# tranqkhue/bugcar_image_segmentation

Hardware: AMD Instinct MI355X
Metric: frames/sec ENet 640x480 segmentation -> BEV occupancy grid (synthetic), whole job (higher is better)
Workload: dtype fp32; 1 GPU; config3/5: ENet 640x480 batch 64 per GPU, preprocess + forward + argmax/LUT + fused BEV warp/occgrid (1000x1000 BEV -> 200x200 cells); global_batch=64, per_gpu_batch=64, height=480, width=640, parallelism=frame-sharded dp1, streams_per_gpu=1, hip_graph=True, ranks=1, devices=1, backend=none (one process)

## Files before the change

### bugcar_image_segmentation_amd/_native.py

```python
from __future__ import annotations

import ctypes
import os
import threading
from pathlib import Path

import torch

_PKG = Path(__file__).resolve().parent
LIB_PATH = Path(os.environ.get("BUGSEG_LIB", _PKG / "libbugseg.so"))

OK, EINVAL, ENOMEM, EHIP, EFORMAT, ESTATE = 0, -1, -2, -3, -4, -5
FP32, BF16, F16 = 0, 1, 2
OUT_LOGITS_F32, OUT_CLASS15_U8, OUT_CLASS3_U8, OUT_BINARY_U8 = 0, 1, 2, 3
PRE_ENGINE, PRE_NCHW_F64, PRE_NCHW_F32, PRE_BGR_U8 = 0, 1, 2, 3

EXPORTED = ("bugseg_version", "bugseg_create", "bugseg_destroy", "bugseg_load_weights", "bugseg_num_classes",
            "bugseg_input_bytes", "bugseg_preprocess", "bugseg_nchw_to_input", "bugseg_enet_forward",
            "bugseg_enet_forward_bgr", "bugseg_enet_forward_bgr_ops", "bugseg_enet_forward_bgr_rows",
            "bugseg_bev_source_rows", "bugseg_debug_row_windows", "bugseg_debug_poison_arena",
            "bugseg_debug_stage3_windows", "bugseg_debug_plan_windows", "bugseg_debug_read_block_output",
            "bugseg_debug_pair_walk", "bugseg_debug_pair_plan",
            "bugseg_bev_occgrid", "bugseg_bev_workspace_bytes", "bugseg_bev_occgrid_ws", "bugseg_plan_info", "bugseg_plan_op", "bugseg_plan_launch_op",
            "bugseg_last_error",
            "bugseg_road_filter_workspace_bytes", "bugseg_road_filter", "bugseg_debug_road_filter_ops",
            "bugseg_clahe_workspace_bytes", "bugseg_clahe_bgr", "bugseg_debug_clahe_stage", "bugseg_debug_clahe_table",
            "bugseg_canny_workspace_bytes", "bugseg_canny", "bugseg_debug_canny_stage", "bugseg_confusion",
            "bugseg_bev_warp_image", "bugseg_hough_trig", "bugseg_hough_workspace_bytes", "bugseg_hough_lines",
            "bugseg_debug_hough_stage",
            "bugseg_quad_workspace_bytes", "bugseg_find_quad", "bugseg_quad_moments", "bugseg_debug_quad_stage",
            "bugseg_map_fuse",
            "bugseg_dl_create", "bugseg_dl_destroy", "bugseg_dl_load_weights", "bugseg_dl_set_plan",
            "bugseg_dl_forward", "bugseg_dl_launch_op", "bugseg_dl_read_buffer", "bugseg_dl_last_error",
            "bugseg_dl_set_class_lut", "bugseg_dl_forward_classes", "bugseg_dl_classes_from_logits",
            "bugseg_debug_parse_pack", "bugseg_debug_polar_tables", "bugseg_debug_ctx_info", "bugseg_debug_tile_walk", "bugseg_debug_set_spans", "bugseg_debug_pool_indices",
            "bugseg_dl_debug_check_plan", "bugseg_debug_knobs", "bugseg_dl_debug_knobs", "bugseg_debug_fused_forms")
DL_OP_FIELDS = 32


class BevParams(ctypes.Structure):
    _fields_ = [("M", ctypes.c_double * 9), ("in_rows", ctypes.c_int), ("in_cols", ctypes.c_int),
                ("warp_w", ctypes.c_int), ("warp_h", ctypes.c_int), ("occ_w_px", ctypes.c_int),
                ("occ_h_px", ctypes.c_int), ("occ_w", ctypes.c_int), ("occ_h", ctypes.c_int),
                ("left_x", ctypes.c_int), ("top_y", ctypes.c_int), ("ros_layout", ctypes.c_int),
                ("variant", ctypes.c_int), ("laserscan", ctypes.c_int)]
# ... 58 lines not shown
        lib = ctypes.CDLL(str(p))
        vp, i, sz, cp = ctypes.c_void_p, ctypes.c_int, ctypes.c_size_t, ctypes.c_char_p
        proto = {
            "bugseg_version": (i, []),
            "bugseg_create": (i, [i, i, ctypes.POINTER(vp)]),
            "bugseg_destroy": (i, [vp]),
            "bugseg_load_weights": (i, [vp, vp, sz]),
            "bugseg_num_classes": (i, [vp]),
            "bugseg_input_bytes": (sz, [vp, i, i, i]),
            "bugseg_preprocess": (i, [vp, vp, i, i, i, i, i, i, vp, vp]),
            "bugseg_nchw_to_input": (i, [vp, vp, i, i, i, i, vp, vp]),
            "bugseg_enet_forward": (i, [vp, vp, i, i, i, i, vp, vp]),
            "bugseg_enet_forward_bgr": (i, [vp, vp, i, i, i, i, vp, vp]),
            "bugseg_enet_forward_bgr_ops": (i, [vp, vp, i, i, i, i, vp, i, i, vp]),
            "bugseg_enet_forward_bgr_rows": (i, [vp, vp, i, i, i, i, vp, i, i, i, i, vp]),
            "bugseg_bev_source_rows": (i, [vp, ctypes.POINTER(BevParams), i, i, ctypes.POINTER(i), ctypes.POINTER(i)]),
            "bugseg_debug_row_windows": (i, [i, i, i, i, i, i, vp]),
            "bugseg_debug_poison_arena": (i, [vp, i, vp]),
            "bugseg_debug_stage3_windows": (i, [i, i, i, i, vp, vp]),
            "bugseg_debug_plan_windows": (i, [vp, i, i, vp]),
            "bugseg_debug_read_block_output": (i, [vp, i, vp, sz, vp]),
            "bugseg_debug_pair_walk": (i, [i, vp, i, i, vp]),
            "bugseg_debug_pair_plan": (i, [vp, vp, i]),
            "bugseg_bev_occgrid": (i, [vp, vp, i, ctypes.POINTER(BevParams), vp, vp]),
            "bugseg_bev_workspace_bytes": (sz, [ctypes.POINTER(BevParams), i]),
            "bugseg_bev_occgrid_ws": (i, [vp, vp, i, ctypes.POINTER(BevParams), vp, vp, sz, vp]),
            "bugseg_plan_info": (i, [vp, i, i, i, i, i, ctypes.POINTER(i), ctypes.POINTER(ctypes.c_double),
                                     ctypes.POINTER(ctypes.c_double), ctypes.POINTER(ctypes.c_double)]),
            "bugseg_plan_op": (i, [vp, i, i, i, i, cp, i, ctypes.POINTER(ctypes.c_double),
                                   ctypes.POINTER(ctypes.c_double), ctypes.POINTER(ctypes.c_double)]),
            "bugseg_plan_launch_op": (i, [vp, i, i, i, i, vp]),
            "bugseg_last_error": (cp, [vp]),
            "bugseg_road_filter_workspace_bytes": (sz, [ctypes.POINTER(RoadFilterParams), i]),
            "bugseg_road_filter": (i, [vp, vp, i, ctypes.POINTER(RoadFilterParams), vp, vp, sz, vp]),
            "bugseg_debug_road_filter_ops": (i, [vp, vp, i, ctypes.POINTER(RoadFilterParams), vp, vp, sz, i, i, vp]),
            "bugseg_clahe_workspace_bytes": (sz, [ctypes.POINTER(ClaheParams), i]),
            "bugseg_clahe_bgr": (i, [vp, vp, i, ctypes.POINTER(ClaheParams), vp, vp, sz, vp]),
            "bugseg_debug_clahe_stage": (i, [vp, vp, i, ctypes.POINTER(ClaheParams), i, vp, vp, sz, vp]),
            "bugseg_debug_clahe_table": (i, [i, vp, sz]),
            "bugseg_canny_workspace_bytes": (sz, [ctypes.POINTER(CannyParams), i]),
            "bugseg_canny": (i, [vp, vp, i, ctypes.POINTER(CannyParams), vp, vp, sz, vp]),
            "bugseg_debug_canny_stage": (i, [vp, vp, i, ctypes.POINTER(CannyParams), i, vp, vp, sz, vp]),
            "bugseg_confusion": (i, [vp, vp, vp, i, ctypes.POINTER(ConfusionParams), vp, vp]),
            "bugseg_bev_warp_image": (i, [vp, vp, i, i, ctypes.POINTER(BevParams), i, vp, vp]),
            "bugseg_hough_trig": (i, [ctypes.POINTER(HoughParams), vp]),
            "bugseg_hough_workspace_bytes": (sz, [ctypes.POINTER(HoughParams), i]),
# ... 68 lines not shown
    if lib.bugseg_debug_fused_forms(rows, n) != n:
        raise RuntimeError("bugseg_debug_fused_forms: the form count changed between two calls")
    return [dict(zip(FORM_COLS, rows[k * len(FORM_COLS):(k + 1) * len(FORM_COLS)])) for k in range(n)]


def tile_walk(ntiles: int, grid: int, rev: int) -> list[list[int]]:
    lib = load_library()
    per_max = (ntiles + 7) // 8
    seq = (ctypes.c_int32 * (grid * per_max))()
    count = (ctypes.c_int32 * grid)()
    per = lib.bugseg_debug_tile_walk(ntiles, grid, rev, seq, len(seq), count)
    if per < 0:
        check(per)
    return [list(seq[b * per:b * per + count[b]]) for b in range(grid)]


def row_windows(H: int, W: int, row0: int, row1: int, tile_rows_c64: int = 8, tile_rows_c16: int = 16) -> list[tuple[int, int]]:
    lib = load_library()
    win = (ctypes.c_int32 * 12)()
    check(lib.bugseg_debug_row_windows(H, W, row0, row1, tile_rows_c64, tile_rows_c16, win))
    return [(win[2 * k], win[2 * k + 1]) for k in range(6)]


def stage3_windows(h: int, y0: int, y1: int, blocks) -> list[tuple[int, int]]:
    lib = load_library()
    flat = [int(v) for b in blocks for v in b]
    blk = (ctypes.c_int32 * max(1, len(flat)))(*flat)
    win = (ctypes.c_int32 * max(1, 2 * len(blocks)))()
    m = lib.bugseg_debug_stage3_windows(h, y0, y1, len(blocks), blk, win)
    if m < 0:
        check(m)
    return [(win[2 * k], win[2 * k + 1]) for k in range(m)]


def pair_walk(cands, first_op: int = 0, last_op: int = -1):
    lib = load_library()
    n = len(cands)
    flat = [int(v) for c in cands for v in c]
    cand = (ctypes.c_int32 * max(1, len(flat)))(*flat)
    out = (ctypes.c_int32 * max(1, 2 * n))()
    m = lib.bugseg_debug_pair_walk(n, cand, first_op, n if last_op < 0 else last_op, out)
    if m < 0:
        check(m)
    return m, [(out[2 * k], out[2 * k + 1]) for k in range(n)]


# ... 68 lines not shown

    def bev_source_rows(self, params: BevParams, rows: int, cols: int) -> tuple[int, int]:
        r0, r1 = ctypes.c_int(0), ctypes.c_int(0)
        check(self.lib.bugseg_bev_source_rows(self.h, ctypes.byref(params), rows, cols, ctypes.byref(r0),
                                              ctypes.byref(r1)), self.h)
        return r0.value, r1.value

    def poison_arena(self, byte: int, stream=None) -> None:
        check(self.lib.bugseg_debug_poison_arena(self.h, int(byte), ctypes.c_void_p(stream_handle(stream))), self.h)

    def plan_windows(self, rows) -> list[tuple[int, int, int, int, int]]:
        win = (ctypes.c_int32 * 10)()
        m = self.lib.bugseg_debug_plan_windows(self.h, int(rows[0]), int(rows[1]), win)
        if m < 0:
            check(m, self.h)
        return [tuple(win[5 * k:5 * k + 5]) for k in range(m)]

    def pair_plan(self) -> list[tuple[int, ...]]:
        rows = (ctypes.c_int32 * (8 * 16))()
        m = self.lib.bugseg_debug_pair_plan(self.h, rows, 16)
        if m < 0:
            check(m, self.h)
        return [tuple(rows[8 * k:8 * k + 8]) for k in range(min(m, 16))]

    def read_block_output(self, op: int, out, stream=None) -> None:
        check(self.lib.bugseg_debug_read_block_output(self.h, op, out.data_ptr(), out.numel() * out.element_size(),
                                                      ctypes.c_void_p(stream_handle(stream))), self.h)

    def _stream_ws(self, x, stream, workspace=None, size_fn=None, params=None, B=0):
        st = stream if stream is not None else torch.cuda.current_stream(x.device)
        ws = workspace
        nws = int(size_fn(ctypes.byref(params), B)) if ws is None and size_fn is not None else 0
        if nws:
            with torch.cuda.stream(st):
                ws = torch.empty(nws, dtype=torch.uint8, device=x.device)
        return stream_handle(st), ((0, 0) if ws is None else (ws.data_ptr(), ws.numel() * ws.element_size())), ws

    def _raise_any(self, rc: int) -> None:
        if rc != OK:
            raise BugsegError(rc, self.lib.bugseg_last_error(self.h).decode(errors="replace"))

    def bev(self, seg, B, params: BevParams, out, stream=None):
        sh, w, _keep = self._stream_ws(seg, stream, None, self.lib.bugseg_bev_workspace_bytes, params, B)
        check(self.lib.bugseg_bev_occgrid_ws(self.h, seg.data_ptr(), B, ctypes.byref(params), out.data_ptr(), *w, sh),
              self.h)

# ... 209 lines not shown
```

### bugcar_image_segmentation_amd/csrc/bugseg_runtime.cpp

```cpp
#include <climits>
#include <cmath>
#include <cstdio>
#include <cstring>
#include <string>
#include <vector>
#include <algorithm>
#include <cstdlib>
#include <mutex>
#include <variant>

#include "bugseg_internal.h"
#include "../../include/bugseg.h"

using namespace bugseg;

namespace {
std::mutex g_occ_mu;
struct OccKey { int dev; const void *f; int threads; size_t lds; int val; };
std::vector<OccKey> g_occ;
int current_device() {
    int d = 0;
    return hipGetDevice(&d) == hipSuccess ? d : 0;
}
}
// ... 21 lines not shown
    const int dev = current_device();
    std::lock_guard<std::mutex> lk(g_occ_mu);
    for (const OccKey &k : g_occ)
        if (k.dev == dev && k.f == f && k.threads == -1) return hipSuccess;
    hipError_t e = hipFuncSetAttribute(f, hipFuncAttributeMaxDynamicSharedMemorySize, 160 * 1024);
    if (e == hipSuccess) g_occ.push_back({dev, f, -1, 0, 1});
    return e;
}

bool bugseg::read_knobs(Knobs &k, std::string &err) {
    k = Knobs();
    auto read = [&](const char *var, int &field, long lo, long hi) {
        const char *v = std::getenv(var);
        if (!v || !*v) return true;
        char *end = nullptr;
        const long n = std::strtol(v, &end, 10);
        const bool ok = (*v == '-' || (*v >= '0' && *v <= '9')) && !*end && n >= lo && n <= hi && !(&field == &k.bev_f && n == 3);
        if (ok) field = (int)n;
        else err = std::string(var) + "=" + v + ": not a decimal integer this knob takes (" + std::to_string(lo) + " to " + std::to_string(hi) + ")";
        return ok;
    };
#define X(name, field, def, lo, hi) if (!read("BUGSEG_" #name, k.field, lo, hi)) return false;
    BUGSEG_KNOBS(X)
#undef X
    return true;
}
int bugseg::dump_knobs(const Knobs *k, char *buf, int len, std::string &err) {
    Knobs now;
    if (!k && !read_knobs(now, err)) return BUGSEG_EINVAL;
    if (!k) k = &now;
    std::string s;
#define X(name, field, def, lo, hi) s += "BUGSEG_" #name "=" + std::to_string(k->field) + "\n";
    BUGSEG_KNOBS(X)
#undef X
    if (!buf || len <= (int)s.size()) {
        err = "the knob dump needs a buffer of " + std::to_string(s.size() + 1) + " bytes";
        return BUGSEG_EINVAL;
    }
    std::memcpy(buf, s.c_str(), s.size() + 1);
    return BUGSEG_OK;
}

int bugseg::range_weight_exp(double m) {
    if (!(m > 0) || !std::isfinite(m)) return 0;
    int e = 0;
    (void)std::frexp(m, &e);
// ... 61 lines not shown
    int fwd_odd = 0;
    double layer() const { return layer_bytes >= 0 ? layer_bytes : bytes; }
    const ConvLaunch *conv() const { return std::get_if<ConvLaunch>(&l); }
    const BneckLaunch *bneck() const { return std::get_if<BneckLaunch>(&l); }
    const UpLaunch *up() const { return std::get_if<UpLaunch>(&l); }
    bool regular(int C, int h) const {
        const BneckLaunch *b = bneck();
        return b && b->C == C && !b->asym && b->cin == 0 && b->a.dt == 1 && b->a.phases == 1 && b->a.H == h;
    }
    bool up_on(int h) const { return up() && up()->a.h == h; }
    bool epi(int e) const { return conv() && conv()->epi == e; }
    bool class_kernel() const { return conv() && conv()->cls; }
};

struct Binding {
    const void *in = nullptr;
    bool bgr = false;
    int out_kind = 0; void *out = nullptr;
};

constexpr int WIN_OPS = 6;
struct WinOp { int y0 = 0, y1 = 0, var = 0, tr = 0, te = 1, tiles_x = 0, tiles_y = 0; Launch l; };
constexpr int S3_OPS = 2;
struct WinPlan {
    int row0 = 0, row1 = 0; WinOp op[WIN_OPS]; int ns3 = 0; WinOp s3[S3_OPS];
    const Launch *launch_of(int i, int n) const {
        const int k = i - (n - WIN_OPS);
        return k >= 0 ? &op[k].l : -k - 1 < ns3 ? &s3[-k - 1].l : nullptr;
    }
};

struct PairCand { bool ok = false; int h = 0, w = 0, in = -1, out = -1; };
std::vector<int> pair_firsts(const std::vector<PairCand> &c) {
    std::vector<int> f;
    for (size_t i = 0; i + 1 < c.size(); ++i) {
        const PairCand &p = c[i], &q = c[i + 1];
        if (p.ok && q.ok && p.h == q.h && p.w == q.w && p.in >= 0 && p.out >= 0 && p.in != p.out && q.in == p.out && q.out == p.in) {
            f.push_back((int)i);
            ++i;
        }
    }
    return f;
}
enum { PA_PLAIN = 0, PA_PAIR = 1, PA_SKIP = 2, PA_LONE_FIRST = 3, PA_LONE_SECOND = 4 };
void pair_actions(int n, const std::vector<int> &firsts, int first_op, int last_op, int *act, int *flip) {
    for (int k = 0; k < n; ++k) { act[k] = PA_PLAIN; flip[k] = 0; }
    for (const int i : firsts) {
        if (i < 0 || i + 1 >= n) continue;
        const bool both = first_op <= i && i + 1 < last_op;
        act[i] = both ? PA_PAIR : PA_LONE_FIRST;
        act[i + 1] = both ? PA_SKIP : PA_LONE_SECOND;
        for (int k = i + 2; k < n; ++k) flip[k] ^= 1;
    }
}
struct PairOp {
    int first = 0, flip = 0;
    BneckPairArgs args{};
    BneckGuardArgs ga{}, gb{};
};

struct Plan {
    int B = 0, H = 0, W = 0;
    std::vector<Op> ops;
    std::vector<int> firsts;
    std::vector<PairOp> pairs;
    std::vector<WinPlan> wins;
    size_t act_bytes = 0;
    float *words = nullptr;
    size_t words_bytes = 0;
    void *arena = nullptr;
    size_t arena_bytes = 0;
    bool pinned = false;
    std::vector<unsigned char *> idx;
    std::vector<size_t> idx_bytes;
    bool cls_ok = false, cls_on = false;
    Launch cls_fused, cls_fused_fwd;
    Binding bound;
};

inline int round_up(int v, int m) { return (v + m - 1) / m * m; }
inline int pow2_nr(int npad) {
    int nr = npad / 16;
    int p = 1;
    while (p < nr) p <<= 1;
    return p;
}

}

// ... 944 lines not shown
    a.cw = l.w; a.cbias = l.bias; a.ncls = l.ncls; a.csw = l.rg.sw[0];
    a.cls_bytes = (uint32_t)((size_t)l.B * l.Hout * l.Wout);
    return f;
}

Launch flipped(const Launch &l, unsigned char *const X[2]) {
    Launch f = l;
    auto mv = [&](auto *&p) {
        using P = std::remove_reference_t<decltype(p)>;
        if ((const void *)p == X[0]) p = (P)X[1];
        else if ((const void *)p == X[1]) p = (P)X[0];
    };
    if (ConvLaunch *c = std::get_if<ConvLaunch>(&f)) { mv(c->a.in); mv(c->a.out); mv(c->a.res); }
    else if (UpLaunch *u = std::get_if<UpLaunch>(&f)) { mv(u->a.x); mv(u->a.out); }
    else if (BneckLaunch *b = std::get_if<BneckLaunch>(&f)) { mv(b->a.x); mv(b->a.out); mv(b->a.xin); }
    return f;
}

void build_pairs(bugseg_ctx *ctx, unsigned char *const X[2], unsigned char *spare, size_t spare_bytes) {
    Plan &pl = ctx->plan;
    const int n = (int)pl.ops.size();
    pl.pairs.clear();
    pl.firsts.clear();
    const Knobs &k = ctx->knobs;
    if (ctx->prec == PREC_F32 && !k.no_fuse && k.bneck_variant < 0 && k.bneck_variant_c64 < 0) {
        auto buf = [&](const void *p) { return p == X[0] ? 0 : p == X[1] ? 1 : -1; };
        std::vector<PairCand> c((size_t)n);
        for (int i = 0; i < n - WIN_OPS; ++i) {
            const BneckLaunch *b = pl.ops[(size_t)i].bneck();
            if (!b || !pl.ops[(size_t)i].regular(64, b->a.H) || b->a.tr || b->cls || b->win || b->var < 0 || b->var > 2) continue;
            if (b->a.x_bytes > spare_bytes) continue;
            c[(size_t)i] = PairCand{true, b->a.H, b->a.W, buf(b->a.x), buf(b->a.out)};
        }
        pl.firsts = pair_firsts(c);
    }
    std::vector<int> act((size_t)n), flip((size_t)n);
    pair_actions(n, pl.firsts, 0, n, act.data(), flip.data());
    for (int i = 0; i < n; ++i) {
        Op &op = pl.ops[(size_t)i];
        op.fwd = flip[(size_t)i] ? flipped(op.l, X) : op.l;
        op.fwd_odd = (op.pos & 1) ^ flip[(size_t)i];
    }
    int th, tw, threads;
    size_t lds;
    bneck_pair_shape(th, tw, threads, lds);
    for (int i = 0; i < n; ++i) {
// ... 81 lines not shown
    pl.act_bytes = total - al(words_bytes);
    pl.wins.clear();
    return true;
}

template <typename F>
void row_windows(int H, int row0, int row1, F tile_rows, int (*win)[2]) {
    const int h2 = H / 2, h4 = H / 4, h8 = H / 8;
    int a = row0, b = row1;
    auto set = [&](int k) { win[k][0] = a; win[k][1] = b; };
    auto halve = [&](int h) { a >>= 1; b = std::min((b + 1) >> 1, h); };
    auto grow = [&](int h) { a = std::max(a - 1, 0); b = std::min(b + 1, h); };
    auto tiles = [&](int k, int h) {
        const int t = std::max(1, tile_rows(k, a, b));
        b = std::min(a + (b - a + t - 1) / t * t, h);
    };
    halve(h2); set(5);
    b = std::min(b + 1, h2);
    tiles(4, h2); set(4); grow(h2);
    halve(h4); set(3);
    tiles(2, h4); set(2); grow(h4);
    tiles(1, h4); set(1); grow(h4);
    halve(h8); set(0);
}

struct S3Desc { int asym = 0, d = 1, rd = 0, rows_full = 0; };
template <typename F>
int stage3_windows(int h, int y0, int y1, int n, const S3Desc *blk, F tile_rows, int (*win)[2]) {
    int a = std::max(y0, 0), b = std::min(y1, h), k = 0;
    for (; k < n; ++k) {
        const S3Desc &q = blk[k];
        if (a >= b || (a == 0 && b == h) || q.d < 1) break;
        int e = b, run;
        if (q.rd) {
            if (q.asym || (q.d & (q.d - 1))) break;
            run = b - a;
        } else {
            if (q.d != 1) break;
            const int t = tile_rows(k, a, b);
            if (t <= 0) break;
            run = (b - a + t - 1) / t * t;
            e = std::min(a + run, h);
        }
        if (run >= q.rows_full) break;
        win[k][0] = a; win[k][1] = e;
        const int reach = q.asym ? 2 : q.d;
// ... 36 lines not shown
        if (w.row0 == row0 && w.row1 == row1) return &w;
    const int n = (int)pl.ops.size(), H = pl.H;
    if (n < WIN_OPS + 1 || pl.cls_ok) return nullptr;
    const Op *o = &pl.ops[(size_t)(n - WIN_OPS)];
    if (!(o[0].up_on(H / 8) && o[1].regular(64, H / 4) && o[2].regular(64, H / 4) && o[3].up_on(H / 4) &&
          o[4].regular(16, H / 2) && o[5].class_kernel() && o[5].conv()->a.Hg == H / 2))
        return nullptr;
    auto s3b = [&](int k) { return n - WIN_OPS - 1 - k >= 0 ? std::get_if<BneckLaunch>(&pl.ops[(size_t)(n - WIN_OPS - 1 - k)].fwd) : nullptr; };
    auto form = [&](const BneckLaunch &q, int rows, bool s3, WinOp &r) {
        auto built = [&](int v) { return !s3 || bneck_slots_per_cu(ctx->knobs, ctx->prec, q.C, q.asym, v, false, 0, true) > 0; };
        int ty = 0, tx = 0, tr = 0, rd = 0;
        int v = pick_bneck_variant(ctx, q.C, q.asym, 1, pl.B, rows, q.a.W, ty, tx, tr, rd);
        if (v < 0 || rd || (s3 && (tr || !built(v)))) { v = q.var; tr = s3 ? 0 : q.a.tr; }
        if (!built(v)) return 0;
        int th, tw, nw;
        bneck_shape(q.C, v, th, tw, nw, nullptr);
        r.var = v; r.tr = tr;
        r.te = tr ? tw : th;
        r.tiles_x = tr ? (q.a.W + th - 1) / th : (q.a.W + tw - 1) / tw;
        return r.te;
    };
    WinPlan w;
    w.row0 = row0; w.row1 = row1;
    int win[WIN_OPS][2];
    row_windows(H, row0, row1, [&](int k, int need0, int need1) { return form(*o[k].bneck(), need1 - need0, false, w.op[k]); }, win);
    for (int k = 0; k < WIN_OPS; ++k) {
        WinOp &r = w.op[k];
        r.y0 = win[k][0]; r.y1 = win[k][1];
        r.tiles_y = (r.y1 - r.y0 + r.te - 1) / r.te;
        r.l = narrow(o[k].fwd, r, false, row0, row1);
    }
    if (ctx->knobs.row_window_s3) {
        S3Desc blk[S3_OPS];
        int nb = 0, th[S3_OPS], tw, nw;
        for (; nb < S3_OPS; ++nb) {
            const BneckLaunch *q = s3b(nb);
            if (!(q && q->C == 128 && q->cin == 0 && q->a.H == H / 8 && q->a.W == o[0].up()->a.w)) break;
            S3Desc &d = blk[nb];
            bneck_shape(128, q->var, th[nb], tw, nw, &d.rd);
            d.asym = q->asym; d.d = q->a.dt;
            d.rows_full = d.rd ? q->a.phases * q->a.tiles_y * th[nb] : q->a.tr ? 0 : q->a.tiles_y * th[nb];
            if (d.rd && bneck_slots_per_cu(ctx->knobs, ctx->prec, 128, false, q->var, false, 0, true) <= 0) d.rows_full = 0;
        }
        int w3[S3_OPS][2];
        w.ns3 = stage3_windows(H / 8, w.op[0].y0, w.op[0].y1, nb, blk,
                               [&](int k, int need0, int need1) { return form(*s3b(k), need1 - need0, true, w.s3[k]); }, w3);
        for (int k = 0; k < w.ns3; ++k) {
            const BneckLaunch &q = *s3b(k);
            WinOp &r = w.s3[k];
            r.y0 = w3[k][0]; r.y1 = w3[k][1];
            if (blk[k].rd) {
                r.var = q.var; r.tr = 0; r.te = th[k]; r.tiles_x = 1;
                r.tiles_y = ((r.y1 - r.y0 + q.a.dt - 1) / q.a.dt + r.te - 1) / r.te;
// ... 259 lines not shown
        }
    }
    hipError_t e = launch_preprocess(a, (hipStream_t)stream);
    if (e != hipSuccess) return fail(ctx, BUGSEG_EHIP, std::string("preprocess launch: ") + hipGetErrorString(e));
    return BUGSEG_OK;
}

int bugseg_nchw_to_input(bugseg_ctx *ctx, const void *x, int is_f64, int B, int H, int W, void *out, void *stream) {
    if (!ctx || !x || !out) return fail(ctx, BUGSEG_EINVAL, "NULL argument");
    if (B <= 0 || H <= 0 || W <= 0) return fail(ctx, BUGSEG_EINVAL, "bad shape");
    DeviceGuard g(ctx->device);
    NchwArgs a{x, is_f64 ? 1 : 0, B, H, W, ctx->prec, out};
    hipError_t e = launch_nchw_to_input(a, (hipStream_t)stream);
    if (e != hipSuccess) return fail(ctx, BUGSEG_EHIP, std::string("layout launch: ") + hipGetErrorString(e));
    return BUGSEG_OK;
}

static hipError_t dispatch(const bugseg_ctx *c, const ConvLaunch &l, hipStream_t s) { return launch_conv(c->prec, l.nr, l.epi, l.a, s, l.cls); }
static hipError_t dispatch(const bugseg_ctx *c, const UpLaunch &l, hipStream_t s) { return launch_up(c->prec, l.cin, l.it, l.cout, l.a, s); }
static hipError_t dispatch(const bugseg_ctx *c, const BneckLaunch &l, hipStream_t s) {
    return l.cls ? launch_bneck_cls(c->knobs, c->prec, l.a, s)
                 : launch_bneck(c->knobs, c->prec, l.C, l.asym, l.var, l.a, s, l.cin, l.win);
}
static int walk_rev(const bugseg_ctx *ctx, int i, bool fwd) {
    const Op &o = ctx->plan.ops[(size_t)i];
    const int order = ctx->knobs.tile_order;
    return order == 2 ? 1 : order == 1 ? (fwd ? o.fwd_odd : o.pos & 1) : 0;
}
static unsigned long long *span_slots(const bugseg_ctx *ctx, int i) {
    return ctx->spans && i < ctx->spans_ops ? ctx->spans + 512 * (size_t)i : nullptr;
}

static hipError_t issue(const bugseg_ctx *ctx, Launch &l, int rev, unsigned long long *span, hipStream_t s) {
    return std::visit([&](auto &r) {
        r.a.span = span;
        r.a.rev = rev;
        return dispatch(ctx, r, s);
    }, l);
}

static void bind(const bugseg_ctx *ctx, const Binding &b, bool first, bool last, Launch &l) {
    ConvLaunch *c = std::get_if<ConvLaunch>(&l);
    if (first && c) {
        c->epi = b.bgr ? EPI_INIT_BGR : EPI_INIT;
        c->a.in = b.in;
        c->a.nlut = b.bgr ? (const double *)((const unsigned char *)ctx->dev_luts + 32) : nullptr;
        c->a.naff_on = b.bgr && ctx->naff_on;
        std::memcpy(c->a.naff, ctx->naff, sizeof(ctx->naff));
        c->a.rg.amax_in = b.bgr ? nullptr : ctx->plan.words;
        c->a.rg.amax_static = b.bgr ? ctx->norm_amax : 0.f;
// ... 1 lines not shown
    if (!last) return;
    const uint8_t *luts = (const uint8_t *)ctx->dev_luts;
    const bool logits = b.out_kind == BUGSEG_OUT_LOGITS_F32;
    uint8_t *cls_out = logits ? nullptr : (uint8_t *)b.out;
    const int lut_kind = b.out_kind == BUGSEG_OUT_CLASS3_U8 ? 1 : b.out_kind == BUGSEG_OUT_BINARY_U8 ? 2 : 0;
    const uint8_t *lut = lut_kind ? luts + 16 * (lut_kind - 1) : nullptr;
    if (BneckLaunch *f = std::get_if<BneckLaunch>(&l)) {
        f->a.cls_out = cls_out; f->a.lut = lut; f->a.lut_kind = lut_kind;
    } else if (c) {
        c->a.cls_out = cls_out; c->a.lut = lut; c->a.lut_kind = lut_kind;
        c->a.logits_out = logits ? (float *)b.out : nullptr;
    }
}

static hipError_t launch_op(const bugseg_ctx *ctx, int i, hipStream_t s, const WinPlan *wp = nullptr, bool fwd = false) {
    const Plan &pl = ctx->plan;
    const int n = (int)pl.ops.size();
    if (pl.cls_on && i + 1 == n) return hipSuccess;
    const bool fused = pl.cls_on && i + 2 == n;
    const Launch *pick = wp ? wp->launch_of(i, n) : nullptr;
    if (!pick) pick = fused ? (fwd ? &pl.cls_fused_fwd : &pl.cls_fused) : fwd ? &pl.ops[(size_t)i].fwd : &pl.ops[(size_t)i].l;
    Launch l = *pick;
    bind(ctx, pl.bound, i == 0, fused || i + 1 == n, l);
    return issue(ctx, l, walk_rev(ctx, i, fwd), span_slots(ctx, i), s);
}

static hipError_t launch_pair(const bugseg_ctx *ctx, const PairOp &p, hipStream_t s) {
    const int i = p.first;
    const BneckLaunch &A = std::get<BneckLaunch>(ctx->plan.ops[(size_t)i].fwd), &Bk = std::get<BneckLaunch>(ctx->plan.ops[(size_t)i + 1].fwd);
    BneckPairArgs a = p.args;
    BneckArgs fa = A.a, fb = Bk.a;
    a.a.rev = fa.rev = walk_rev(ctx, i, true);
    a.a.span = span_slots(ctx, i); fa.span = nullptr;
    fb.rev = walk_rev(ctx, i + 1, true);
    fb.span = span_slots(ctx, i + 1);
    hipError_t e = launch_bneck_pair(ctx->knobs, a, s);
    if (e == hipSuccess) e = launch_bneck_guarded(ctx->knobs, A.var, fa, p.ga, s);
    if (e == hipSuccess) e = launch_bneck_guarded(ctx->knobs, Bk.var, fb, p.gb, s);
    return e;
}

static int enet_forward(bugseg_ctx *ctx, const void *in, bool bgr, int B, int H, int W, int out_kind, void *out,
                        void *stream, int first_op = 0, int last_op = -1, int row0 = 0, int row1 = 0) {
    if (!ctx || !in || !out) return fail(ctx, BUGSEG_EINVAL, "NULL argument");
    if (!ctx->loaded) return fail(ctx, BUGSEG_ESTATE, "no weights loaded");
    if (out_kind < BUGSEG_OUT_LOGITS_F32 || out_kind > BUGSEG_OUT_BINARY_U8) return fail(ctx, BUGSEG_EINVAL, "bad out_kind");
    DeviceGuard g(ctx->device);
    std::string why;
    if (!build_plan(ctx, B, H, W, why, stream)) return fail(ctx, BUGSEG_EINVAL, why);
    Plan &pl = ctx->plan;
    if (stream_capturing(stream)) pl.pinned = true;
    pl.bound = Binding{in, bgr, out_kind, out};
    const int nops = (int)pl.ops.size();
    if (last_op < 0 || last_op > nops) last_op = nops;
    if (first_op < 0 || first_op > last_op) return fail(ctx, BUGSEG_EINVAL, "bad op range");
    if (pl.words && first_op == 0) {
        hipError_t e = hipMemsetAsync(pl.words, 0, pl.words_bytes, (hipStream_t)stream);
        if (e == hipSuccess && !bgr) e = launch_amax((const float *)in, (size_t)B * H * W * 8, pl.words, (hipStream_t)stream);
        if (e != hipSuccess) return fail(ctx, BUGSEG_EHIP, std::string("range words: ") + hipGetErrorString(e));
    }
    pl.cls_on = pl.cls_ok && out_kind != BUGSEG_OUT_LOGITS_F32 && first_op <= nops - 2 && last_op == nops;
    const WinPlan *wp = window_plan(ctx, row0, row1);
    std::vector<int> act(2 * (size_t)nops);
    pair_actions(nops, pl.firsts, first_op, last_op, act.data(), act.data() + nops);
    for (int i = first_op; i < last_op; ++i) {
        hipError_t e = hipSuccess;
        switch (act[(size_t)i]) {
        case PA_SKIP: break;
        case PA_PAIR:
            e = launch_pair(ctx, pl.pairs[(size_t)(std::lower_bound(pl.firsts.begin(), pl.firsts.end(), i) - pl.firsts.begin())], (hipStream_t)stream);
            if (e != hipSuccess) return fail(ctx, BUGSEG_EHIP, "pair launch " + std::to_string(i) + ": " + hipGetErrorString(e));
            break;
        default:
            e = launch_op(ctx, i, (hipStream_t)stream, wp, true);
            if (e != hipSuccess) return fail(ctx, BUGSEG_EHIP, "conv launch " + std::to_string(i) + ": " + hipGetErrorString(e));
        }
    }
    return BUGSEG_OK;
}

int bugseg_enet_forward(bugseg_ctx *ctx, const void *in, int B, int H, int W, int out_kind, void *out, void *stream) {
    return enet_forward(ctx, in, false, B, H, W, out_kind, out, stream);
}

int bugseg_enet_forward_bgr(bugseg_ctx *ctx, const uint8_t *bgr, int B, int H, int W, int out_kind, void *out,
                            void *stream) {
    return enet_forward(ctx, bgr, true, B, H, W, out_kind, out, stream);
}

// ... 417 lines not shown
    }
    return per;
}

int bugseg_debug_fused_forms(int32_t *rows, int n_rows) {
    if (n_rows < 0 || (!rows && n_rows > 0)) return fail(nullptr, BUGSEG_EINVAL, "fused forms: NULL rows");
    const int nb = bneck_form_rows(rows, n_rows);
    const int left = n_rows > nb ? n_rows - nb : 0;
    return nb + up_form_rows(left ? rows + (size_t)nb * FORM_COLS : nullptr, left);
}

int bugseg_debug_row_windows(int H, int W, int row0, int row1, int tile_rows_c64, int tile_rows_c16, int32_t *win) {
    (void)W;
    if (!win) return fail(nullptr, BUGSEG_EINVAL, "NULL argument");
    if (H <= 0 || H % 8 || W <= 0 || W % 8) return fail(nullptr, BUGSEG_EINVAL, "H and W must be positive multiples of 8");
    if (row0 < 0 || row1 > H || row0 >= row1) return fail(nullptr, BUGSEG_EINVAL, "row windows: 0 <= row0 < row1 <= H");
    if (tile_rows_c64 <= 0 || tile_rows_c16 <= 0) return fail(nullptr, BUGSEG_EINVAL, "row windows: tile rows must be positive");
    int w[WIN_OPS][2];
    row_windows(H, row0, row1, [&](int k, int, int) { return k == 4 ? tile_rows_c16 : tile_rows_c64; }, w);
    for (int k = 0; k < WIN_OPS; ++k) { win[2 * k] = w[k][0]; win[2 * k + 1] = w[k][1]; }
    return BUGSEG_OK;
}

int bugseg_debug_poison_arena(bugseg_ctx *ctx, int byte, void *stream) {
    if (!ctx) return fail(ctx, BUGSEG_EINVAL, "NULL ctx");
    Plan &pl = ctx->plan;
    if (!pl.arena) return fail(ctx, BUGSEG_ESTATE, "no forward has run");
    DeviceGuard g(ctx->device);
    hipError_t e = hipMemsetAsync(pl.arena, byte & 255, pl.act_bytes, (hipStream_t)stream);
    if (e != hipSuccess) return fail(ctx, BUGSEG_EHIP, std::string("poison arena: ") + hipGetErrorString(e));
    return BUGSEG_OK;
}

int bugseg_debug_stage3_windows(int h, int y0, int y1, int n, const int32_t *blk, int32_t *win) {
    if (h <= 0 || y0 < 0 || y0 >= y1 || y1 > h || n < 0 || n > 16 || (n && (!blk || !win)))
        return fail(nullptr, BUGSEG_EINVAL, "bad stage-3 walk");
    S3Desc d[16];
    int te[16], w[16][2];
    for (int k = 0; k < n; ++k) {
        d[k].asym = blk[5 * k]; d[k].d = blk[5 * k + 1]; d[k].rd = blk[5 * k + 2]; d[k].rows_full = blk[5 * k + 3];
        te[k] = blk[5 * k + 4];
    }
    const int m = stage3_windows(h, y0, y1, n, d, [&](int k, int, int) { return te[k]; }, w);
    for (int k = 0; k < m; ++k) { win[2 * k] = w[k][0]; win[2 * k + 1] = w[k][1]; }
    return m;
}
// ... 172 lines not shown
```

### bugcar_image_segmentation_amd/csrc/knobs.h

```cpp
#pragma once
#include <string>

#ifndef BUGSEG_TILE_ORDER_DEFAULT
#define BUGSEG_TILE_ORDER_DEFAULT 1
#endif

namespace bugseg {

#define BUGSEG_KNOBS(X) \
    X(F32_RANGE, f32_range, 1, 0, 1) X(NO_PAIR, no_pair, 0, 0, 1) X(NO_FUSE, no_fuse, 0, 0, 1) \
    X(BNECK_VARIANT, bneck_variant, -1, 0, 5) X(BNECK_VARIANT_C128, bneck_variant_c128, -1, 0, bneck_variants(128) - 1) \
    X(BNECK_VARIANT_C64, bneck_variant_c64, -1, 0, bneck_variants(64) - 1) \
    X(BNECK_VARIANT_C16, bneck_variant_c16, -1, 0, bneck_variants(16) - 1) X(BNECK_VARIANT_ASYM, bneck_variant_asym, -1, 0, 5) \
    X(BNECK2, bneck2, 0, 0, 1) X(TILE_ORDER, tile_order, BUGSEG_TILE_ORDER_DEFAULT, 0, 2) X(CLS_FUSE, cls_fuse, 0, 0, 1) \
    X(CLS_CONV, cls_conv, 0, 0, 1) X(ROW_WINDOW_S3, row_window_s3, 1, 0, 1) X(INIT_TABLE, init_table, 0, 0, 1) \
    X(INIT_POOL_SCAN, init_pool_scan, 0, 0, 1) X(BNECK_GRID, bneck_grid, 0, INT_MIN, INT_MAX) \
    X(BEV_F, bev_f, 0, 1, 4)  X(BEV_FG, bev_fg, 0, 0, INT_MAX) X(BEV_BAND, bev_band, 1, 0, 1) \
    X(BEV_FB, bev_fb, 1, 1, 2) X(BEV_NEAR_FIRST, bev_near_first, 0, 0, 1) \
    X(DL_GEMM, dl_gemm, 1, 0, 1) X(DL_G128, dl_g128, 1, 0, 1) X(DL_IG, dl_ig, 1, 0, 1) X(DL_IG64, dl_ig64, 1, 0, 1) \
    X(DL_GTM, dl_gtm, -1, 0, 1) X(DL_GROUP, dl_group, 1, 0, 1)

struct Knobs {
#define X(name, field, def, lo, hi) int field = def;
    BUGSEG_KNOBS(X)
#undef X
};

bool read_knobs(Knobs &k, std::string &err);
int dump_knobs(const Knobs *k, char *buf, int len, std::string &err);

}
```

### include/bugseg.h

```cpp
#ifndef BUGSEG_H
#define BUGSEG_H

#include <stddef.h>
#include <stdint.h>

#ifdef __cplusplus
extern "C" {
#endif

typedef struct bugseg_ctx bugseg_ctx;

enum {
    BUGSEG_OK = 0,
    BUGSEG_EINVAL = -1,
    BUGSEG_ENOMEM = -2,
    BUGSEG_EHIP = -3,
    BUGSEG_EFORMAT = -4,
    BUGSEG_ESTATE = -5
};

enum { BUGSEG_FP32 = 0, BUGSEG_BF16 = 1, BUGSEG_F16 = 2 };

enum {
    BUGSEG_OUT_LOGITS_F32 = 0,
// ... 155 lines not shown

int bugseg_confusion(bugseg_ctx *ctx, const uint8_t *pred_dev, const uint8_t *gt_dev, int B,
                     const bugseg_confusion_params *p, int64_t *acc_dev, void *stream);

int bugseg_plan_info(bugseg_ctx *ctx, int B, int H, int W, int out_kind, int bgr_input, int *n_launches,
                     double *alg_bytes, double *plan_bytes, double *flops);

int bugseg_plan_op(bugseg_ctx *ctx, int B, int H, int W, int op, char *kernel, int kernel_len, double *alg_bytes,
                   double *plan_bytes, double *flops);
int bugseg_plan_launch_op(bugseg_ctx *ctx, int B, int H, int W, int op, void *stream);

const char *bugseg_last_error(const bugseg_ctx *ctx);

int bugseg_debug_parse_pack(const void *blob, size_t bytes, int precision, int *ncls);
int bugseg_debug_polar_tables(int w, int h, int variant, int32_t *fmap, size_t fmap_n, int32_t *imap, size_t imap_n,
                              int *pw, int *ph);
int bugseg_debug_tile_walk(int ntiles, int grid, int rev, int32_t *seq, size_t seq_n, int32_t *count);
int bugseg_debug_row_windows(int H, int W, int row0, int row1, int tile_rows_c64, int tile_rows_c16, int32_t *win);
int bugseg_debug_stage3_windows(int h, int y0, int y1, int n, const int32_t *blk, int32_t *win);
int bugseg_debug_plan_windows(bugseg_ctx *ctx, int row0, int row1, int32_t *win);
int bugseg_debug_read_block_output(bugseg_ctx *ctx, int op, void *dst_dev, size_t bytes, void *stream);
int bugseg_debug_pair_walk(int n, const int32_t *cand, int first_op, int last_op, int32_t *out);
int bugseg_debug_pair_plan(bugseg_ctx *ctx, int32_t *rows, int cap);
int bugseg_debug_poison_arena(bugseg_ctx *ctx, int byte, void *stream);
int bugseg_debug_ctx_info(const bugseg_ctx *ctx, int what, int arg);
int bugseg_debug_knobs(const bugseg_ctx *ctx, char *buf, int len);
int bugseg_debug_fused_forms(int32_t *rows, int n_rows);
int bugseg_debug_set_spans(bugseg_ctx *ctx, void *spans, int n_ops);
int bugseg_debug_pool_indices(bugseg_ctx *ctx, int B, int H, int W, int block, void *dst, size_t bytes, int *idx_cs,
                              void *stream);

#define BUGSEG_DL_OP_FIELDS 32
typedef struct bugseg_dl bugseg_dl;

int bugseg_dl_create(int device, int precision, bugseg_dl **out);
int bugseg_dl_destroy(bugseg_dl *dl);
int bugseg_dl_load_weights(bugseg_dl *dl, const void *blob, size_t bytes);
int bugseg_dl_set_plan(bugseg_dl *dl, const int32_t *ops, int nops, const uint64_t *buf_bytes, int nbufs,
                       int B, int Hc, int Wc);
int bugseg_dl_forward(bugseg_dl *dl, const uint8_t *rgb_dev, int B, int H, int W, int64_t *out_dev, void *stream);
int bugseg_dl_set_class_lut(bugseg_dl *dl, const uint8_t *lut, int n);
int bugseg_dl_forward_classes(bugseg_dl *dl, const uint8_t *img_dev, int bgr, int B, int H, int W, uint8_t *seg_dev,
                              int row0, int row1, void *stream);
int bugseg_dl_classes_from_logits(bugseg_dl *dl, int B, int H, int W, uint8_t *seg_dev, int row0, int row1,
                                  void *stream);
int bugseg_dl_launch_op(bugseg_dl *dl, int op, void *stream);
// ... 11 lines not shown
```

Before: 23770 frames/s.

## Fuse two decoder bottlenecks into a paired launch inside the row-window plan

Extends the row-windowed (BEV source rows) forward plan so that two consecutive decoder bottleneck ops (ops 1 and 2 of the window) run as one fused pair kernel. The intermediate goes through a spare buffer, and the following ops have their ping-pong buffers flipped. The row window for the pair is rounded up to the pair tile height, and the upstream window is widened to cover it. The aim is to cut one launch and the round trip of the intermediate activation through global memory, at the cost of some extra rows computed from the rounding and more complex buffer aliasing.

```diff
diff --git a/bugcar_image_segmentation_amd/_native.py b/bugcar_image_segmentation_amd/_native.py
--- a/bugcar_image_segmentation_amd/_native.py
+++ b/bugcar_image_segmentation_amd/_native.py
@@ -20,7 +20,7 @@
             "bugseg_enet_forward_bgr", "bugseg_enet_forward_bgr_ops", "bugseg_enet_forward_bgr_rows",
             "bugseg_bev_source_rows", "bugseg_debug_row_windows", "bugseg_debug_poison_arena",
             "bugseg_debug_stage3_windows", "bugseg_debug_plan_windows", "bugseg_debug_read_block_output",
-            "bugseg_debug_pair_walk", "bugseg_debug_pair_plan",
+            "bugseg_debug_pair_walk", "bugseg_debug_pair_plan", "bugseg_debug_row_windows_pair", "bugseg_debug_decoder_pair",
             "bugseg_bev_occgrid", "bugseg_bev_workspace_bytes", "bugseg_bev_occgrid_ws", "bugseg_plan_info", "bugseg_plan_op", "bugseg_plan_launch_op",
             "bugseg_last_error",
             "bugseg_road_filter_workspace_bytes", "bugseg_road_filter", "bugseg_debug_road_filter_ops",
@@ -125,6 +125,8 @@
             "bugseg_debug_read_block_output": (i, [vp, i, vp, sz, vp]),
             "bugseg_debug_pair_walk": (i, [i, vp, i, i, vp]),
             "bugseg_debug_pair_plan": (i, [vp, vp, i]),
+            "bugseg_debug_row_windows_pair": (i, [i, i, i, i, i, i, i, vp]),
+            "bugseg_debug_decoder_pair": (i, [vp, i, i, vp]),
             "bugseg_bev_occgrid": (i, [vp, vp, i, ctypes.POINTER(BevParams), vp, vp]),
             "bugseg_bev_workspace_bytes": (sz, [ctypes.POINTER(BevParams), i]),
             "bugseg_bev_occgrid_ws": (i, [vp, vp, i, ctypes.POINTER(BevParams), vp, vp, sz, vp]),
@@ -239,6 +241,14 @@
     return [(win[2 * k], win[2 * k + 1]) for k in range(6)]
 
 
+def row_windows_pair(H: int, W: int, row0: int, row1: int, tile_rows_c64: int = 8, tile_rows_c16: int = 16,
+                     pair_rows: int = 12) -> list[tuple[int, int]]:
+    lib = load_library()
+    win = (ctypes.c_int32 * 14)()
+    check(lib.bugseg_debug_row_windows_pair(H, W, row0, row1, tile_rows_c64, tile_rows_c16, pair_rows, win))
+    return [(win[2 * k], win[2 * k + 1]) for k in range(7)]
+
+
 def stage3_windows(h: int, y0: int, y1: int, blocks) -> list[tuple[int, int]]:
     lib = load_library()
     flat = [int(v) for b in blocks for v in b]
@@ -353,6 +363,13 @@
         if m < 0:
             check(m, self.h)
         return [tuple(rows[8 * k:8 * k + 8]) for k in range(min(m, 16))]
+
+    def decoder_pair(self, rows) -> tuple[int, ...] | None:
+        info = (ctypes.c_int32 * 8)()
+        m = self.lib.bugseg_debug_decoder_pair(self.h, int(rows[0]), int(rows[1]), info)
+        if m < 0:
+            check(m, self.h)
+        return tuple(info) if m else None
 
     def read_block_output(self, op: int, out, stream=None) -> None:
         check(self.lib.bugseg_debug_read_block_output(self.h, op, out.data_ptr(), out.numel() * out.element_size(),
diff --git a/bugcar_image_segmentation_amd/csrc/bugseg_runtime.cpp b/bugcar_image_segmentation_amd/csrc/bugseg_runtime.cpp
--- a/bugcar_image_segmentation_amd/csrc/bugseg_runtime.cpp
+++ b/bugcar_image_segmentation_amd/csrc/bugseg_runtime.cpp
@@ -67,6 +67,7 @@
     };
 #define X(name, field, def, lo, hi) if (!read("BUGSEG_" #name, k.field, lo, hi)) return false;
     BUGSEG_KNOBS(X)
+    BUGSEG_KNOBS_UNLISTED(X)
 #undef X
     return true;
 }
@@ -174,12 +175,20 @@
 constexpr int WIN_OPS = 6;
 struct WinOp { int y0 = 0, y1 = 0, var = 0, tr = 0, te = 1, tiles_x = 0, tiles_y = 0; Launch l; };
 constexpr int S3_OPS = 2;
+struct PairOp {
+    int first = 0, flip = 0;
+    BneckPairArgs args{};
+    BneckGuardArgs ga{}, gb{};
+};
 struct WinPlan {
     int row0 = 0, row1 = 0; WinOp op[WIN_OPS]; int ns3 = 0; WinOp s3[S3_OPS];
     const Launch *launch_of(int i, int n) const {
         const int k = i - (n - WIN_OPS);
         return k >= 0 ? &op[k].l : -k - 1 < ns3 ? &s3[-k - 1].l : nullptr;
     }
+    bool paired = false;
+    PairOp pair;
+    int py0 = 0, py1 = 0, pth = 0, ptw = 0;
 };
 
 struct PairCand { bool ok = false; int h = 0, w = 0, in = -1, out = -1; };
@@ -205,18 +214,14 @@
         for (int k = i + 2; k < n; ++k) flip[k] ^= 1;
     }
 }
-struct PairOp {
-    int first = 0, flip = 0;
-    BneckPairArgs args{};
-    BneckGuardArgs ga{}, gb{};
-};
-
 struct Plan {
     int B = 0, H = 0, W = 0;
     std::vector<Op> ops;
     std::vector<int> firsts;
     std::vector<PairOp> pairs;
     std::vector<WinPlan> wins;
+    unsigned char *X[2] = {nullptr, nullptr}, *spare = nullptr;
+    size_t spare_bytes = 0;
     size_t act_bytes = 0;
     float *words = nullptr;
     size_t words_bytes = 0;
@@ -1207,6 +1212,7 @@
     const int n = (int)pl.ops.size();
     pl.pairs.clear();
     pl.firsts.clear();
+    pl.X[0] = X[0]; pl.X[1] = X[1]; pl.spare = spare; pl.spare_bytes = spare_bytes;
     const Knobs &k = ctx->knobs;
     if (ctx->prec == PREC_F32 && !k.no_fuse && k.bneck_variant < 0 && k.bneck_variant_c64 < 0) {
         auto buf = [&](const void *p) { return p == X[0] ? 0 : p == X[1] ? 1 : -1; };
@@ -1334,6 +1340,17 @@
     tiles(2, h4); set(2); grow(h4);
     tiles(1, h4); set(1); grow(h4);
     halve(h8); set(0);
+}
+
+template <typename F>
+void row_windows_pair(int H, int row0, int row1, int pair_rows, F tile_rows, int (*win)[2]) {
+    row_windows(H, row0, row1, tile_rows, win);
+    const int h4 = H / 4, h8 = H / 8, t = std::max(1, pair_rows);
+    const int a = win[3][0], b = win[3][1];
+    win[6][0] = a; win[6][1] = std::min(a + (b - a + t - 1) / t * t, h4);
+    const int lo = std::max(std::min(win[6][0] - 2, win[1][0] - 1), 0);
+    const int hi = std::min(std::max(win[6][1] + 2, win[1][1] + 1), h4);
+    win[0][0] = lo >> 1; win[0][1] = std::min((hi + 1) >> 1, h8);
 }
 
 struct S3Desc { int asym = 0, d = 1, rd = 0, rows_full = 0; };
@@ -1416,13 +1433,48 @@
     };
     WinPlan w;
     w.row0 = row0; w.row1 = row1;
-    int win[WIN_OPS][2];
-    row_windows(H, row0, row1, [&](int k, int need0, int need1) { return form(*o[k].bneck(), need1 - need0, false, w.op[k]); }, win);
+    int win[WIN_OPS + 1][2];
+    auto rows_of = [&](int k, int need0, int need1) { return form(*o[k].bneck(), need1 - need0, false, w.op[k]); };
+    row_windows(H, row0, row1, rows_of, win);
+    const Knobs &kn = ctx->knobs;
+    const BneckLaunch &A = std::get<BneckLaunch>(o[1].fwd), &Bk = std::get<BneckLaunch>(o[2].fwd);
+    int pth = 0;
+    if (ctx->prec == PREC_F32 && !kn.no_fuse && kn.bneck_variant < 0 && kn.bneck_variant_c64 < 0 && kn.pair_decoder &&
+        !A.a.tr && !Bk.a.tr && !A.cls && !Bk.cls && !A.win && !Bk.win && A.a.W == Bk.a.W && A.a.x_bytes <= pl.spare_bytes &&
+        (A.a.x == pl.X[0] || A.a.x == pl.X[1]) && (A.a.out == pl.X[0] || A.a.out == pl.X[1]) && A.a.x != A.a.out &&
+        Bk.a.x == A.a.out && Bk.a.out == A.a.x && !w.op[1].tr && !w.op[2].tr && w.op[1].var >= 0 && w.op[1].var <= 2 &&
+        w.op[2].var >= 0 && w.op[2].var <= 2) {
+        int tw, threads;
+        size_t lds;
+        bneck_pair_shape(pth, tw, threads, lds);
+    }
+    if (pth) row_windows_pair(H, row0, row1, pth, rows_of, win);
     for (int k = 0; k < WIN_OPS; ++k) {
         WinOp &r = w.op[k];
         r.y0 = win[k][0]; r.y1 = win[k][1];
         r.tiles_y = (r.y1 - r.y0 + r.te - 1) / r.te;
         r.l = narrow(o[k].fwd, r, false, row0, row1);
+    }
+    if (pth) {
+        int th, tw, threads;
+        size_t lds;
+        bneck_pair_shape(th, tw, threads, lds);
+        BneckLaunch fa = A, fb = Bk;
+        PairOp &p = w.pair;
+        p.first = n - WIN_OPS + 1; p.flip = 0;
+        p.args.a = A.a; p.args.b = Bk.a;
+        p.args.b.out = A.a.out;
+        p.args.a.oy_base = win[WIN_OPS][0];
+        p.args.a.tiles_y = (win[WIN_OPS][1] - win[WIN_OPS][0] + th - 1) / th; p.args.a.tiles_x = (A.a.W + tw - 1) / tw;
+        p.args.a.ntiles = A.a.B * p.args.a.tiles_y * p.args.a.tiles_x;
+        p.ga.ra = A.a.rg; p.ga.rb = Bk.a.rg; p.ga.clear = Bk.a.rg.amax_out;
+        p.gb = p.ga; p.gb.clear = nullptr;
+        fa.a.out = pl.spare;
+        fb.a.x = pl.spare; fb.a.out = p.args.b.out;
+        w.op[1].l = narrow(Launch(fa), w.op[1], false, row0, row1);
+        w.op[2].l = narrow(Launch(fb), w.op[2], false, row0, row1);
+        for (int k = 3; k < WIN_OPS; ++k) w.op[k].l = narrow(flipped(o[k].fwd, pl.X), w.op[k], false, row0, row1);
+        w.paired = true; w.py0 = win[WIN_OPS][0]; w.py1 = win[WIN_OPS][1]; w.pth = th; w.ptw = tw;
     }
     if (ctx->knobs.row_window_s3) {
         S3Desc blk[S3_OPS];
@@ -1728,10 +1780,11 @@
     return l.cls ? launch_bneck_cls(c->knobs, c->prec, l.a, s)
                  : launch_bneck(c->knobs, c->prec, l.C, l.asym, l.var, l.a, s, l.cin, l.win);
 }
-static int walk_rev(const bugseg_ctx *ctx, int i, bool fwd) {
+static int walk_rev(const bugseg_ctx *ctx, int i, bool fwd, const WinPlan *wp = nullptr) {
     const Op &o = ctx->plan.ops[(size_t)i];
     const int order = ctx->knobs.tile_order;
-    return order == 2 ? 1 : order == 1 ? (fwd ? o.fwd_odd : o.pos & 1) : 0;
+    const int behind = fwd && wp && wp->paired && i > wp->pair.first + 1 ? 1 : 0;
+    return order == 2 ? 1 : order == 1 ? (fwd ? o.fwd_odd ^ behind : o.pos & 1) : 0;
 }
 static unsigned long long *span_slots(const bugseg_ctx *ctx, int i) {
     return ctx->spans && i < ctx->spans_ops ? ctx->spans + 512 * (size_t)i : nullptr;
@@ -1779,12 +1832,13 @@
     if (!pick) pick = fused ? (fwd ? &pl.cls_fused_fwd : &pl.cls_fused) : fwd ? &pl.ops[(size_t)i].fwd : &pl.ops[(size_t)i].l;
     Launch l = *pick;
     bind(ctx, pl.bound, i == 0, fused || i + 1 == n, l);
-    return issue(ctx, l, walk_rev(ctx, i, fwd), span_slots(ctx, i), s);
-}
-
-static hipError_t launch_pair(const bugseg_ctx *ctx, const PairOp &p, hipStream_t s) {
+    return issue(ctx, l, walk_rev(ctx, i, fwd, wp), span_slots(ctx, i), s);
+}
+
+static hipError_t launch_pair(const bugseg_ctx *ctx, const PairOp &p, hipStream_t s, const WinPlan *wp = nullptr) {
     const int i = p.first;
-    const BneckLaunch &A = std::get<BneckLaunch>(ctx->plan.ops[(size_t)i].fwd), &Bk = std::get<BneckLaunch>(ctx->plan.ops[(size_t)i + 1].fwd);
+    const BneckLaunch &A = std::get<BneckLaunch>(wp ? wp->op[1].l : ctx->plan.ops[(size_t)i].fwd);
+    const BneckLaunch &Bk = std::get<BneckLaunch>(wp ? wp->op[2].l : ctx->plan.ops[(size_t)i + 1].fwd);
     BneckPairArgs a = p.args;
     BneckArgs fa = A.a, fb = Bk.a;
     a.a.rev = fa.rev = walk_rev(ctx, i, true);
@@ -1820,8 +1874,15 @@
     const WinPlan *wp = window_plan(ctx, row0, row1);
     std::vector<int> act(2 * (size_t)nops);
     pair_actions(nops, pl.firsts, first_op, last_op, act.data(), act.data() + nops);
+    const int dpair = wp && wp->paired ? wp->pair.first : -1;
     for (int i = first_op; i < last_op; ++i) {
         hipError_t e = hipSuccess;
+        if (i == dpair && i + 1 < last_op) {
+            e = launch_pair(ctx, wp->pair, (hipStream_t)stream, wp);
+            if (e != hipSuccess) return fail(ctx, BUGSEG_EHIP, "pair launch " + std::to_string(i) + ": " + hipGetErrorString(e));
+            ++i;
+            continue;
+        }
         switch (act[(size_t)i]) {
         case PA_SKIP: break;
         case PA_PAIR:
@@ -2285,6 +2346,31 @@
     return BUGSEG_OK;
 }
 
+int bugseg_debug_row_windows_pair(int H, int W, int row0, int row1, int tile_rows_c64, int tile_rows_c16, int pair_rows,
+                                  int32_t *win) {
+    (void)W;
+    if (!win) return fail(nullptr, BUGSEG_EINVAL, "NULL argument");
+    if (H <= 0 || H % 8 || W <= 0 || W % 8) return fail(nullptr, BUGSEG_EINVAL, "H and W must be positive multiples of 8");
+    if (row0 < 0 || row1 > H || row0 >= row1) return fail(nullptr, BUGSEG_EINVAL, "row windows: 0 <= row0 < row1 <= H");
+    if (tile_rows_c64 <= 0 || tile_rows_c16 <= 0 || pair_rows <= 0) return fail(nullptr, BUGSEG_EINVAL, "row windows: tile rows must be positive");
+    int w[WIN_OPS + 1][2];
+    row_windows_pair(H, row0, row1, pair_rows, [&](int k, int, int) { return k == 4 ? tile_rows_c16 : tile_rows_c64; }, w);
+    for (int k = 0; k <= WIN_OPS; ++k) { win[2 * k] = w[k][0]; win[2 * k + 1] = w[k][1]; }
+    return BUGSEG_OK;
+}
+
+int bugseg_debug_decoder_pair(bugseg_ctx *ctx, int row0, int row1, int32_t *info) {
+    if (!ctx || !info) return fail(ctx, BUGSEG_EINVAL, "NULL argument");
+    if (!ctx->plan.arena) return fail(ctx, BUGSEG_ESTATE, "no forward has run");
+    DeviceGuard g(ctx->device);
+    const WinPlan *wp = window_plan(ctx, row0, row1);
+    if (!wp || !wp->paired) return 0;
+    const BneckArgs &a = wp->pair.args.a;
+    const int32_t v[8] = {wp->pair.first, wp->py0, wp->py1, wp->pth, wp->ptw, a.tiles_y, a.tiles_x, a.ntiles};
+    std::memcpy(info, v, sizeof(v));
+    return 1;
+}
+
 int bugseg_debug_poison_arena(bugseg_ctx *ctx, int byte, void *stream) {
     if (!ctx) return fail(ctx, BUGSEG_EINVAL, "NULL ctx");
     Plan &pl = ctx->plan;
diff --git a/bugcar_image_segmentation_amd/csrc/knobs.h b/bugcar_image_segmentation_amd/csrc/knobs.h
--- a/bugcar_image_segmentation_amd/csrc/knobs.h
+++ b/bugcar_image_segmentation_amd/csrc/knobs.h
@@ -20,9 +20,12 @@
     X(DL_GEMM, dl_gemm, 1, 0, 1) X(DL_G128, dl_g128, 1, 0, 1) X(DL_IG, dl_ig, 1, 0, 1) X(DL_IG64, dl_ig64, 1, 0, 1) \
     X(DL_GTM, dl_gtm, -1, 0, 1) X(DL_GROUP, dl_group, 1, 0, 1)
 
+#define BUGSEG_KNOBS_UNLISTED(X) X(PAIR_DECODER, pair_decoder, 1, 0, 1)
+
 struct Knobs {
 #define X(name, field, def, lo, hi) int field = def;
     BUGSEG_KNOBS(X)
+    BUGSEG_KNOBS_UNLISTED(X)
 #undef X
 };
 
diff --git a/include/bugseg.h b/include/bugseg.h
--- a/include/bugseg.h
+++ b/include/bugseg.h
@@ -201,6 +201,9 @@
 int bugseg_debug_read_block_output(bugseg_ctx *ctx, int op, void *dst_dev, size_t bytes, void *stream);
 int bugseg_debug_pair_walk(int n, const int32_t *cand, int first_op, int last_op, int32_t *out);
 int bugseg_debug_pair_plan(bugseg_ctx *ctx, int32_t *rows, int cap);
+int bugseg_debug_row_windows_pair(int H, int W, int row0, int row1, int tile_rows_c64, int tile_rows_c16, int pair_rows,
+                                  int32_t *win);
+int bugseg_debug_decoder_pair(bugseg_ctx *ctx, int row0, int row1, int32_t *info);
 int bugseg_debug_poison_arena(bugseg_ctx *ctx, int byte, void *stream);
 int bugseg_debug_ctx_info(const bugseg_ctx *ctx, int what, int arg);
 int bugseg_debug_knobs(const bugseg_ctx *ctx, char *buf, int len);
```

Result: no change. 23980 frames/s, median of 6 (+0.9%).
